# SonyCSLParis/audio-metrics

Hardware: AMD Instinct MI355X
Metric: evaluate() embeddings/sec (FAD+KD+PRDC), 2×100k CLAP-512 sets, 1/2/4/8 GPUs (higher is better)
Workload: dtype f32

## Files before the change

audio-metrics_amd/_lib.py:

```python
import ctypes
import os
from ctypes import c_char_p, c_double, c_int, c_int64, c_size_t, c_void_p

from ._build import DEV_LIB_PATH, LIB_PATH

_P = c_void_p

SIGNATURES = {
    "am_version": (c_char_p, []),
    "am_status_string": (c_char_p, [c_int]),
    "am_last_error": (c_char_p, []),
    "am_stats_workspace_bytes": (c_size_t, [c_int64, c_int]),
    "am_stats_f32": (c_int, [_P, c_int64, c_int, c_int64, _P, _P, _P, c_size_t, _P]),
    "am_colsum_f32": (c_int, [_P, c_int64, c_int, c_int64, _P, _P, c_size_t, _P]),
    "am_scatter_f32": (c_int, [_P, c_int64, c_int, c_int64, _P, _P, _P, c_size_t, _P]),
    "am_stats_f64_workspace_bytes": (c_size_t, [c_int64, c_int]),
    "am_stats_f64": (c_int, [_P, c_int64, c_int, c_int64, _P, _P, _P, c_size_t, _P]),
    "am_colsum_f64": (c_int, [_P, c_int64, c_int, c_int64, _P, _P, c_size_t, _P]),
    "am_scatter_f64": (c_int, [_P, c_int64, c_int, c_int64, _P, _P, _P, c_size_t, _P]),
    "am_stats_merge_f64": (c_int, [c_int64, _P, _P, c_int64, _P, _P, c_int, _P, _P, _P]),
    "am_stats_push_max_rows": (c_int, []),
    "am_stats_push_f32": (c_int, [_P, c_int64, c_int, c_int64, c_int64, _P, _P, _P, _P, c_int64, _P]),
    "am_frechet_workspace_bytes": (c_size_t, [c_int]),
    "am_frechet_f64": (c_int, [_P, _P, _P, _P, c_int, c_int, c_double, _P, _P, c_size_t, _P]),
    "am_frechet_first_block": (c_int, []),
    "am_frechet_enqueue_f64": (c_int, [_P, _P, _P, _P, c_int, c_int, c_int, c_int, c_double, _P, _P, c_size_t, _P]),
    "am_apa_f64": (c_double, [c_double, c_double, c_double]),
    "am_kd_workspace_bytes": (c_size_t, [c_int, c_int]),
    "am_kd_poly_workspace_bytes": (c_size_t, [c_int, c_int, c_int]),
    "am_kd_poly_f32": (c_int, [_P, c_int64, c_int64, _P, c_int64, c_int64, c_int, _P, _P, c_int, c_int,
                               c_double, c_double, c_int, _P, _P, c_size_t, _P]),
    "am_kd_draw_indices": (c_int, [ctypes.c_uint64, ctypes.c_uint64, ctypes.c_uint64, ctypes.c_uint64, c_int64, c_int64, c_int,
                                   c_int, _P, _P]),
    "am_kd_rbf_workspace_bytes": (c_size_t, [c_int, c_int]),
    "am_kd_rbf_f32": (c_int, [_P, c_int64, c_int64, _P, c_int64, c_int64, c_int, _P, _P, c_int, c_int, c_double, _P, _P,
                              c_size_t, _P]),
    "am_knn_workspace_bytes": (c_size_t, [c_int64, c_int64, c_int, c_int]),
    "am_knn_radii_f32": (c_int, [_P, c_int64, c_int64, _P, c_int64, c_int64, c_int, c_int, _P, _P, c_size_t, _P]),
    "am_knn_sym_eligible": (c_int, [c_int64, c_int, c_int]),
    "am_knn_list_width": (c_int, [c_int]),
    "am_knn_part_workspace_bytes": (c_size_t, [c_int64, c_int, c_int]),
    "am_knn_bounds_f32": (c_int, [_P, c_int64, c_int64, c_int, c_int, c_int64, c_int64, _P, _P, c_size_t, _P]),
    "am_knn_sym_part_f32": (c_int, [_P, c_int64, c_int64, c_int, c_int, c_int, c_int, _P, _P, _P, c_size_t, _P]),
    "am_knn_lists_finish_workspace_bytes": (c_size_t, [c_int64, c_int, c_int]),
    "am_knn_lists_finish_f32": (c_int, [_P, c_int, _P, c_int64, c_int64, c_int, c_int, _P, _P, c_size_t, _P]),
    "am_prdc_workspace_bytes": (c_size_t, [c_int64, c_int64, c_int]),
    "am_prdc_counts_f32": (c_int, [_P, c_int64, c_int64, _P, c_int64, c_int64, c_int, _P, _P, _P, _P, _P, _P,
                                   _P, c_size_t, _P]),
    "am_prdc_reduce": (c_int, [_P, c_int64, _P, _P, c_int64, _P, _P]),
    "am_prepared_half_ld": (c_int64, [c_int]),
    "am_prepare_set_f32": (c_int, [_P, c_int64, c_int64, c_int, _P, _P, _P, _P]),
    "am_knn_radii_prepared_f32": (c_int, [_P, c_int64, c_int64, c_int, _P, c_int, _P, _P, c_size_t, _P]),
    "am_knn_bounds_prepared_f32": (c_int, [_P, c_int64, c_int64, c_int, _P, c_int, c_int64, c_int64, _P, _P, c_size_t, _P]),
    "am_knn_sym_part_prepared_f32": (c_int, [_P, c_int64, c_int64, c_int, _P, c_int, c_int, c_int, _P, _P, _P, c_size_t, _P]),
    "am_prdc_counts_prepared_f32": (c_int, [_P, c_int64, c_int64, _P, _P, c_int64, c_int64, _P, c_int, _P, _P, _P, _P, _P, _P,
                                            _P, c_size_t, _P]),
    "am_knn_f64_workspace_bytes": (c_size_t, [c_int64, c_int64, c_int, c_int]),
    "am_knn_radii_f64": (c_int, [_P, c_int64, c_int64, _P, c_int64, c_int64, c_int, c_int, _P, _P, c_size_t, _P]),
    "am_prdc_f64_workspace_bytes": (c_size_t, [c_int64, c_int64, c_int]),
    "am_prdc_counts_f64": (c_int, [_P, c_int64, c_int64, _P, c_int64, c_int64, c_int, _P, _P, _P, _P, _P, _P,
                                   _P, c_size_t, _P]),
    "am_kd_f64_workspace_bytes": (c_size_t, [c_int, c_int]),
    "am_kd_poly_f64": (c_int, [_P, c_int64, c_int64, _P, c_int64, c_int64, c_int, _P, _P, c_int, c_int,
                               c_double, c_double, c_int, _P, _P, c_size_t, _P]),
    "am_kd_rbf_f64": (c_int, [_P, c_int64, c_int64, _P, c_int64, c_int64, c_int, _P, _P, c_int, c_int, c_double, _P, _P,
                              c_size_t, _P]),
    "am_eigh_workspace_bytes": (c_size_t, [c_int]),
    "am_eigh_sym_f64": (c_int, [_P, c_int, _P, _P, c_int, _P, c_size_t, _P]),
    "am_project_f64": (c_int, [_P, c_int64, c_int64, c_int, _P, _P, c_int, _P, _P]),
    "am_project_rows_f64": (c_int, [_P, c_int64, c_int64, c_int, _P, _P, c_int, _P, _P]),
    "am_evaluate_workspace_bytes": (c_size_t, [c_int64, c_int64, c_int, c_int, c_int, c_int, ctypes.c_uint]),
    "am_evaluate_f32": (c_int, [_P, c_int64, c_int64, _P, c_int64, c_int64, c_int, ctypes.c_uint, c_int, _P, _P, c_int, c_int,
                                c_double, c_double, c_int, _P, _P, _P, _P, c_size_t, _P, _P]),
    "am_evaluate_sharded_workspace_bytes": (c_size_t, [_P, _P, c_int, c_int, c_int, c_int, c_int, c_int, ctypes.c_uint]),
    "am_evaluate_sharded_f32": (c_int, [_P, c_int64, _P, c_int64, c_int, _P, _P, _P, ctypes.c_uint, c_int, _P, _P, c_int, c_int,
                                        c_double, c_double, c_int, _P, _P, c_size_t, _P, _P, _P]),
    "am_kernel_clock_enable": (c_int, [c_int]),
    "am_kernel_clock_read": (c_int, [c_int, _P, _P]),
    "am_knn_path": (c_int, [c_int64, c_int64, c_int, c_int, c_int]),
    "am_prdc_path": (c_int, [c_int64, c_int64, c_int]),
    "am_kd_path": (c_int, [c_int64, c_int64, c_int64, c_int64, c_int, c_int, c_int, c_int]),
    "am_filter_engine": (c_int, [c_int]),
    "am_filter_stats_enable": (c_int, [_P]),
}


class HipLibraryError(RuntimeError):
    pass


class PreparedSetStruct(ctypes.Structure):
    _fields_ = [("norms", c_void_p), ("stats", c_void_p), ("half", c_void_p)]


class EvaluateSideStruct(ctypes.Structure):
    _fields_ = [("mean", c_void_p), ("cov", c_void_p), ("radii", c_void_p),
                ("mean_out", c_void_p), ("cov_out", c_void_p), ("radii_out", c_void_p)]


ALL_REDUCE_SUM_FN = ctypes.CFUNCTYPE(c_int, c_void_p, c_void_p, c_int64, c_int, c_void_p)
ALL_GATHER_V_FN = ctypes.CFUNCTYPE(c_int, c_void_p, c_void_p, c_void_p, ctypes.POINTER(c_int64), c_void_p)


class CollectivesStruct(ctypes.Structure):
# ... 43 lines not shown
```

audio-metrics_amd/csrc/am_common.h:

```cpp
#pragma once
#include <hip/hip_runtime.h>
#include <stdint.h>
#include <stddef.h>
#include <stdio.h>
#include "../../include/audio_metrics_hip.h"

namespace am {

char* last_error_buf();
void set_error(const char* fmt, ...);

#define AM_HIP_TRY(expr)                                                             \
    do {                                                                             \
        hipError_t _e = (expr);                                                      \
        if (_e != hipSuccess) {                                                      \
            am::set_error("%s failed: %s (%s:%d)", #expr, hipGetErrorString(_e),     \
                          __FILE__, __LINE__);                                       \
            return AM_ERR_HIP;                                                       \
        }                                                                            \
    } while (0)

#define AM_LAUNCH_CHECK()                                                            \
    do {                                                                             \
        hipError_t _e = hipGetLastError();                                           \
        if (_e != hipSuccess) {                                                      \
            am::set_error("kernel launch failed: %s (%s:%d)", hipGetErrorString(_e), \
                          __FILE__, __LINE__);                                       \
            return AM_ERR_HIP;                                                       \
        }                                                                            \
    } while (0)

#define AM_REQUIRE(cond, status, ...)                                                \
    do {                                                                             \
        if (!(cond)) {                                                               \
            am::set_error(__VA_ARGS__);                                              \
            return (status);                                                         \
        }                                                                            \
    } while (0)

hipError_t ensure_dynamic_lds(const void* kernel, int bytes);

void clock_begin(int kernel, hipStream_t st);
void clock_end(int kernel, hipStream_t st);

__device__ __forceinline__ float clamp0(float v) { return v != v ? __builtin_inff() : fmaxf(v, 0.f); }

static inline bool aligned16(const void* p) { return (reinterpret_cast<uintptr_t>(p) & 15u) == 0; }
static inline size_t round_up(size_t x, size_t a) { return (x + a - 1) / a * a; }
static inline int64_t ceil_div(int64_t a, int64_t b) { return (a + b - 1) / b; }

struct Carver {
    char* base;
    size_t size;
    size_t off = 0;
    Carver(void* p, size_t n) : base(static_cast<char*>(p)), size(n) {}
    template <class T>
    T* take(size_t count) {
        size_t bytes = round_up(count * sizeof(T), 256);
        T* r = (base && off + bytes <= size) ? reinterpret_cast<T*>(base + off) : nullptr;
        off += bytes;
        return r;
    }
    bool ok() const { return base != nullptr && off <= size; }
};

bool knn64_filter_eligible(int64_t N, int D, int k);
size_t knn64_filter_workspace(int64_t N, int D, int k);
int knn64_filter(const double* X, int64_t N, int64_t ld, int D, int k, double* out_r, void* ws, size_t ws_bytes, hipStream_t st);
bool prdc64_filter_eligible(int64_t Nr, int64_t Nc, int D);
size_t prdc64_filter_workspace(int64_t Nr, int64_t Nc, int D);
int prdc64_filter(const double* R, int64_t Nr, int64_t ldr, const double* C, int64_t Nc, int64_t ldc, int D, const double* rt,
                  const double* ct, int32_t* col_count, unsigned* row_any, unsigned* row_cover, const int** fail_flag, void* ws,
                  size_t ws_bytes, hipStream_t st);
size_t knn64_self_workspace(int64_t N, int k);
int knn64_self_gated(const double* X, int64_t N, int64_t ld, int D, int k, double* out_r, void* ws, size_t ws_bytes, const int* run_flag,
                     hipStream_t st);


}
```

audio-metrics_amd/csrc/evaluate.hip:

```cpp
#include "am_common.h"
#include <algorithm>
#include <vector>

namespace am {

__global__ void eval_pack_kernel(const double* __restrict__ fad5, const long long* __restrict__ totals, double* __restrict__ out,
                                 unsigned what) {
    const int t = threadIdx.x;
    if (t < AM_EVAL_HEAD) {
        double v = 0.0;
        if (t < 5) v = (what & AM_EVAL_FAD) ? fad5[t] : (t == 4 ? -1.0 : 0.0);
        else if (t < 9) v = (what & AM_EVAL_PRDC) ? (double)totals[t - 5] : 0.0;
        out[t] = v;
    }
}

struct EvalLayout {
    size_t total = 0;
    size_t stats_ws = 0, knn_ws = 0, prdc_ws = 0, kd_ws = 0, fad_ws = 0;
    double *mean[2] = {nullptr, nullptr}, *cov[2] = {nullptr, nullptr};
    float *norms[2] = {nullptr, nullptr}, *radii[2] = {nullptr, nullptr};
    uint32_t* pstats[2] = {nullptr, nullptr};
    uint16_t* half[2] = {nullptr, nullptr};
    int32_t* col = nullptr;
// ... 32 lines not shown
        main_bytes = std::max({main_bytes, am_knn_workspace_bytes(n_ref, n_ref, D, k), am_knn_workspace_bytes(n_cand, n_cand, D, k),
                               am_prdc_workspace_bytes(n_ref, n_cand, D)});
    }
    if (what & AM_EVAL_KD) main_bytes = std::max(main_bytes, am_kd_poly_workspace_bytes(S, m, D));
    L.ws_main_bytes = round_up(std::max<size_t>(main_bytes, 256), 256);
    L.ws_main = c.take<char>(L.ws_main_bytes);
    L.total = c.off;
    return c.ok();
}

}

using namespace am;

extern "C" size_t am_evaluate_workspace_bytes(int64_t n_ref, int64_t n_cand, int D, int nearest_k, int kd_subsets, int kd_m,
                                              unsigned what) {
    if (n_ref < 1 || n_cand < 1 || D < 1) return 0;
    Carver c(nullptr, 0);
    EvalLayout L;
    eval_layout(c, n_ref, n_cand, D, nearest_k, kd_subsets, kd_m, what, L);
    return L.total;
}

extern "C" int am_evaluate_f32(const float* ref, int64_t n_ref, int64_t ld_ref, const float* cand, int64_t n_cand,
                               int64_t ld_cand, int D, unsigned what, int nearest_k, const int64_t* idx_cand,
                               const int64_t* idx_ref, int kd_subsets, int kd_m, double kd_gamma, double kd_coef0, int kd_degree,
                               const am_evaluate_side* given_ref, const am_evaluate_side* given_cand, double* out, void* ws,
                               size_t ws_bytes, am_stream_t stream, am_stream_t side_stream) {
    AM_REQUIRE(ref && cand && out, AM_ERR_BAD_ARG, "null pointer");
    AM_REQUIRE(n_ref >= 1 && n_cand >= 1 && D >= 1, AM_ERR_BAD_SHAPE, "sets of %lld and %lld rows x %d", (long long)n_ref,
               (long long)n_cand, D);
    AM_REQUIRE((what & ~(unsigned)(AM_EVAL_FAD | AM_EVAL_KD | AM_EVAL_PRDC)) == 0 && what != 0, AM_ERR_BAD_ARG, "what = %u", what);
    AM_REQUIRE(!(what & AM_EVAL_KD) || (idx_cand && idx_ref && kd_subsets >= 1 && kd_m >= 1), AM_ERR_BAD_ARG,
               "kernel distance needs the two index tables");
    AM_REQUIRE(!(what & AM_EVAL_FAD) || side_stream != stream, AM_ERR_BAD_ARG,
               "the Frechet solve runs on side_stream, which must differ from stream");
    hipStream_t st = static_cast<hipStream_t>(stream), side = static_cast<hipStream_t>(side_stream);
#ifdef AM_DEV_KNOBS
    static const int fad_place = getenv("AM_EVAL_FAD_PLACE") ? atoi(getenv("AM_EVAL_FAD_PLACE")) : 0;
#else
    constexpr int fad_place = 0;
#endif
    Carver c(ws, ws_bytes);
    EvalLayout L;
    AM_REQUIRE(eval_layout(c, n_ref, n_cand, D, nearest_k, kd_subsets, kd_m, what, L), AM_ERR_WORKSPACE,
               "workspace too small: need %zu bytes, have %zu", L.total, ws_bytes);
    const float* X[2] = {ref, cand};
    const int64_t n[2] = {n_ref, n_cand}, ld[2] = {ld_ref, ld_cand};
    const am_evaluate_side* given[2] = {given_ref, given_cand};
    int rc;

    const double* mean[2];
    const double* cov[2];
    if (what & AM_EVAL_FAD) {
        for (int s = 0; s < 2; ++s) {
            if (given[s] && given[s]->mean && given[s]->cov) {
                mean[s] = given[s]->mean;
                cov[s] = given[s]->cov;
                continue;
            }
            double* m_out = given[s] && given[s]->mean_out ? given[s]->mean_out : L.mean[s];
            double* c_out = given[s] && given[s]->cov_out ? given[s]->cov_out : L.cov[s];
            if ((rc = am_stats_f32(X[s], n[s], D, ld[s], m_out, c_out, L.ws_main, L.ws_main_bytes, stream)) != AM_OK) return rc;
            mean[s] = m_out;
            cov[s] = c_out;
        }
    }
    struct EventGuard {
        hipEvent_t e = nullptr;
        ~EventGuard() {
            if (e) (void)hipEventDestroy(e);
        }
    } ev_stats, ev_fad;
    if ((what & AM_EVAL_FAD) && fad_place != 2) {
        AM_HIP_TRY(hipEventCreateWithFlags(&ev_stats.e, hipEventDisableTiming));
        AM_HIP_TRY(hipEventRecord(ev_stats.e, st));
    }

    if (what & AM_EVAL_PRDC) {
        am_prepared_set prep[2];
        for (int s = 0; s < 2; ++s) {
            if ((rc = am_prepare_set_f32(X[s], n[s], ld[s], D, L.norms[s], L.pstats[s], L.half[s], stream)) != AM_OK) return rc;
            prep[s].norms = L.norms[s];
            prep[s].stats = L.pstats[s];
            prep[s].half = L.half[s];
        }
        const float* radii[2];
        for (int s = 0; s < 2; ++s) {
            if (given[s] && given[s]->radii) {
                radii[s] = given[s]->radii;
                continue;
            }
            float* r_out = given[s] && given[s]->radii_out ? given[s]->radii_out : L.radii[s];
            if ((rc = am_knn_radii_prepared_f32(X[s], n[s], ld[s], D, &prep[s], nearest_k, r_out, L.ws_main, L.ws_main_bytes,
                                                stream)) != AM_OK)
                return rc;
            radii[s] = r_out;
            if ((what & AM_EVAL_FAD) && fad_place == 2 && ev_stats.e == nullptr) {
                AM_HIP_TRY(hipEventCreateWithFlags(&ev_stats.e, hipEventDisableTiming));
                AM_HIP_TRY(hipEventRecord(ev_stats.e, st));
            }
        }
        if ((rc = am_prdc_counts_prepared_f32(ref, n_ref, ld_ref, &prep[0], cand, n_cand, ld_cand, &prep[1], D, radii[0], radii[1],
                                              L.col, L.rany, L.rcov, nullptr, L.ws_main, L.ws_main_bytes, stream)) != AM_OK)
            return rc;
        if ((rc = am_prdc_reduce(L.col, n_cand, L.rany, L.rcov, n_ref, reinterpret_cast<int64_t*>(L.totals), stream)) != AM_OK)
            return rc;
    }

    if (what & AM_EVAL_KD) {
        if ((rc = am_kd_poly_f32(cand, n_cand, ld_cand, ref, n_ref, ld_ref, D, idx_cand, idx_ref, kd_subsets, kd_m, kd_gamma,
                                 kd_coef0, kd_degree, out + AM_EVAL_HEAD, L.ws_main, L.ws_main_bytes, stream)) != AM_OK)
            return rc;
    }

    if (what & AM_EVAL_FAD) {
        const bool serial = fad_place == 1;
        if (!serial) {
            if (ev_stats.e == nullptr) {
                AM_HIP_TRY(hipEventCreateWithFlags(&ev_stats.e, hipEventDisableTiming));
                AM_HIP_TRY(hipEventRecord(ev_stats.e, st));
            }
            AM_HIP_TRY(hipStreamWaitEvent(side, ev_stats.e, 0));
        }
        const int block = am_frechet_first_block(), max_iter = 64;
        for (int first = 0; first < 2 * block; first += block)
            if ((rc = am_frechet_enqueue_f64(mean[1], cov[1], mean[0], cov[0], D, first, block, max_iter, 1e-13, L.fad_out,
                                             L.ws_fad, L.fad_ws, serial ? stream : side_stream)) != AM_OK)
                return rc;
        if (!serial) {
            AM_HIP_TRY(hipEventCreateWithFlags(&ev_fad.e, hipEventDisableTiming));
            AM_HIP_TRY(hipEventRecord(ev_fad.e, side));
            AM_HIP_TRY(hipStreamWaitEvent(st, ev_fad.e, 0));
        }
    }
// ... 358 lines not shown
```

audio-metrics_amd/csrc/pairwise.hip:

```cpp
#include "pairwise_common.h"
#include <algorithm>
#include <vector>
#include <cmath>
#include <type_traits>

namespace am {

__global__ void __launch_bounds__(256) row_sqnorm_kernel(const float* __restrict__ X, int64_t N, int64_t ld,
                                                         int D, float* __restrict__ out) {
    const int lane = threadIdx.x & 63;
    const int64_t row = (int64_t)blockIdx.x * 4 + (threadIdx.x >> 6);
    if (row >= N) return;
    const float* x = X + row * ld;
    float acc = 0.f;
    for (int k = lane * 4; k < D; k += 256) {
        const f32x4 v = load_k4(x, k, D);
        acc = fmaf(v.x, v.x, acc);
        acc = fmaf(v.y, v.y, acc);
        acc = fmaf(v.z, v.z, acc);
        acc = fmaf(v.w, v.w, acc);
    }
#pragma unroll
    for (int off = 32; off >= 1; off >>= 1) acc = acc + __shfl_xor(acc, off);
    if (lane == 0) out[row] = acc;
// ... 1261 lines not shown
    L.c32 = c.take<float>((size_t)Nc * L.ld32);
    L.rn = c.take<float>(Nr);
    L.rt = c.take<float>(Nr);
    L.cn = c.take<float>(Nc);
    L.ct = c.take<float>(Nc);
    L.rmin = c.take<unsigned>(Nr);
    L.plan = plan_cross_fast(Nr, Nc, D);
    L.buf = carve_cross_fast(c, Nr, Nc, D, L.plan);
    L.total = c.off;
    return c.ok();
}
size_t prdc64_filter_workspace(int64_t Nr, int64_t Nc, int D) {
    Carver c(nullptr, 0);
    Prdc64Layout L;
    prdc64_layout(c, Nr, Nc, D, L);
    return L.total;
}

int prdc64_filter(const double* R, int64_t Nr, int64_t ldr, const double* C, int64_t Nc, int64_t ldc, int D, const double* rt,
                  const double* ct, int32_t* col_count, unsigned* row_any, unsigned* row_cover, const int** fail_flag, void* ws,
                  size_t ws_bytes, hipStream_t st) {
    Carver c(ws, ws_bytes);
    Prdc64Layout L;
    AM_REQUIRE(prdc64_layout(c, Nr, Nc, D, L), AM_ERR_WORKSPACE, "workspace too small: need %zu bytes, have %zu", L.total, ws_bytes);
    hipLaunchKernelGGL(cast64_kernel, dim3((unsigned)ceil_div(Nr * L.ld32, 256)), dim3(256), 0, st, R, Nr, ldr, D, L.r32, L.ld32);
    hipLaunchKernelGGL(cast64_kernel, dim3((unsigned)ceil_div(Nc * L.ld32, 256)), dim3(256), 0, st, C, Nc, ldc, D, L.c32, L.ld32);
    hipLaunchKernelGGL(narrow64_kernel, dim3((unsigned)ceil_div(Nr, 256)), dim3(256), 0, st, rt, Nr, L.rt);
    hipLaunchKernelGGL(narrow64_kernel, dim3((unsigned)ceil_div(Nc, 256)), dim3(256), 0, st, ct, Nc, L.ct);
    hipLaunchKernelGGL(fill_u32_kernel, dim3((unsigned)ceil_div(Nr, 256)), dim3(256), 0, st, L.rmin, Nr, 0x7f800000u);
    AM_LAUNCH_CHECK();
    int rc;
    if ((rc = norms_of(nullptr, L.r32, Nr, L.ld32, D, L.rn, st)) != AM_OK) return rc;
    if ((rc = norms_of(nullptr, L.c32, Nc, L.ld32, D, L.cn, st)) != AM_OK) return rc;
    const Prdc64Hook h{R, C, ldr, ldc, rt, ct};
    if ((rc = run_cross_fast(L.r32, Nr, L.ld32, L.rn, L.rt, L.c32, Nc, L.ld32, L.cn, L.ct, D, L.plan, L.buf, col_count, L.rmin, row_any,
                             row_cover, false, st, nullptr, nullptr, &h)) != AM_OK)
        return rc;
    *fail_flag = L.buf.ov_count + 1;
    return AM_OK;
}

}

extern "C" int am_knn_radii_f32(const float* X, int64_t N, int64_t ldx, const float* Y, int64_t M, int64_t ldy,
                                int D, int k, float* out_r, void* ws, size_t ws_bytes, am_stream_t stream) {
    return knn_radii_impl(X, N, ldx, Y, M, ldy, D, k, out_r, ws, ws_bytes, stream, nullptr);
}

static bool prepared_ok(const am_prepared_set* p) { return p != nullptr && p->norms != nullptr && p->stats != nullptr && p->half != nullptr; }
static PreparedSet prepared_of(const am_prepared_set* p) { return PreparedSet{p->norms, p->stats, p->half}; }

extern "C" int64_t am_prepared_half_ld(int D) { return D < 1 ? 0 : half_ld(D); }

extern "C" int am_prepare_set_f32(const float* X, int64_t N, int64_t ld, int D, float* norms, uint32_t* stats4, uint16_t* half,
                                  am_stream_t stream) {
    int rc;
    if ((rc = check_matrix(X, N, ld, D, "X")) != AM_OK) return rc;
    AM_REQUIRE(norms && stats4 && half, AM_ERR_BAD_ARG, "null output pointer");
    hipStream_t st = static_cast<hipStream_t>(stream);
    if ((rc = launch_norms(X, N, ld, D, norms, st)) != AM_OK) return rc;
    AM_HIP_TRY(hipMemsetAsync(stats4, 0, 4 * sizeof(unsigned), st));
    return launch_to_half(X, N, ld, D, norms, stats4, 0, half, st);
}

extern "C" int am_knn_radii_prepared_f32(const float* X, int64_t N, int64_t ldx, int D, const am_prepared_set* prepared, int k,
                                         float* out_r, void* ws, size_t ws_bytes, am_stream_t stream) {
    AM_REQUIRE(prepared_ok(prepared), AM_ERR_BAD_ARG, "prepared set has a null member");
    const PreparedSet ps = prepared_of(prepared);
    return knn_radii_impl(X, N, ldx, X, N, ldx, D, k, out_r, ws, ws_bytes, stream, &ps);
}

extern "C" int am_filter_stats_enable(int64_t* device_slots) {
    if (device_slots == nullptr) {
        g_filter_stats = nullptr;
        g_filter_stats_device = -1;
        return AM_OK;
    }
    int dev = -1;
    AM_HIP_TRY(hipGetDevice(&dev));
    g_filter_stats = reinterpret_cast<long long*>(device_slots);
    g_filter_stats_device = dev;
    return AM_OK;
}

extern "C" int am_knn_path(int64_t N, int64_t M, int D, int k, int self) {
    if (N < 1 || M < 1 || D < 1 || k < 1) return -1;
    if (k > AM_MAX_K) return 4;
    const KnnPlan p = plan_knn(N, M, D, k, self != 0 && N == M);
    return !p.sym ? 0 : (knn_fast_enabled(N, D) ? (p.tile_rows == 256 ? 3 : 2) : 1);
}
extern "C" int am_prdc_path(int64_t Nr, int64_t Nc, int D) {
    if (Nr < 1 || Nc < 1 || D < 1) return -1;
    if (!cross_fast_enabled(Nr, Nc, D)) return 0;
    return plan_cross_fast(Nr, Nc, D).wide ? 3 : 2;
}

extern "C" int am_filter_engine(int D) {
    if (D < 1) return 0;
    const int Dh = (int)(half_ld(D) / 2);
    return wide_stationary(Dh) ? (pstat64_supported(Dh) ? 2 : 1) : 0;
}

extern "C" int am_knn_sym_eligible(int64_t N, int D, int k) {
    if (N < 1 || D < 1 || k < 1 || k > AM_MAX_K) return 0;
    return plan_knn(N, N, D, k, true).sym ? 1 : 0;
}

extern "C" int am_knn_list_width(int k) { return (k < 1 || k > AM_MAX_K) ? 0 : kcap_for(k + 1); }

extern "C" size_t am_knn_part_workspace_bytes(int64_t N, int D, int k) {
    if (N < 1 || D < 1 || k < 1 || k > AM_MAX_K) return 0;
    const KnnPlan p = plan_knn(N, N, D, k, true, true);
    Carver c(nullptr, 0);
    KnnBuffers b;
    carve_knn(c, N, N, p, b);
// ... 313 lines not shown
```

audio-metrics_amd/csrc/stats.hip:

```cpp
#include "am_common.h"
#include "tile_engine.h"
#include <algorithm>

namespace am {

constexpr int SC_ROWS = 32;
constexpr int SC_LD = 128;
constexpr int SC_SLAB = SC_ROWS * SC_LD;
constexpr int SC_FLUSH = 8;

__global__ void __launch_bounds__(256) colsum_partial_kernel(const float* __restrict__ X, int64_t N, int64_t ld,
                                                             int D, int64_t rows_per_block,
                                                             double* __restrict__ partial) {
    __shared__ double red[256 * 4];
    const int tid = threadIdx.x;
    const int cgs = (D + 3) / 4;
    const int cpp = cgs < 256 ? cgs : 256;
    const int rpar = 256 / cpp;
    const int my_cg = tid % cpp, my_r = tid / cpp;
    const int64_t r0 = (int64_t)blockIdx.x * rows_per_block;
    const int64_t r1 = (r0 + rows_per_block < N) ? r0 + rows_per_block : N;
    for (int cg0 = 0; cg0 < cgs; cg0 += cpp) {
        const int cg = cg0 + my_cg;
        double s0 = 0, s1 = 0, s2 = 0, s3 = 0;
// ... 260 lines not shown
        mu[which][c] = s / (double)b;
    }
    __syncthreads();
    for (int e = tid; e < b * PUSH_TILE; e += 256) {
        const int r = e / PUSH_TILE, c = e % PUSH_TILE;
        ea[r][c] -= (float)mu[0][c];
        eb[r][c] -= (float)mu[1][c];
    }
    __syncthreads();
    const double n1 = (double)n_old, n2 = (double)b, n = n1 + n2;
    const int c = tid % PUSH_TILE;
#pragma unroll
    for (int q = 0; q < PUSH_TILE / 8; ++q) {
        const int r = tid / PUSH_TILE + 8 * q;
        const int gi = i0 + r, gj = j0 + c;
        if (gi >= D || gj >= D) continue;
        double sum = 0;
        for (int k = 0; k < b; ++k) sum = fma((double)ea[k][r], (double)eb[k][c], sum);
        const double cov2 = b > 1 ? sum / (double)(b - 1) : 0.0;
        const int64_t o = (int64_t)gi * D + gj;
        if (n_old == 0) {
            cov[o] = cov2;
        } else {
            const double w1 = (n1 - 1) / (n - 1), w2 = (n2 - 1) / (n - 1), wd = (n1 * n2 / n) / (n - 1);
            const double di = mean_in[gi] - mu[0][r], dj = mean_in[gj] - mu[1][c];
            cov[o] = (w1 * cov[o] + w2 * cov2) + wd * (di * dj);
        }
    }
    if (ti == tj && tid < PUSH_TILE && i0 + tid < D) {
        const int g = i0 + tid;
        mean_out[g] = n_old == 0 ? mu[0][tid] : (n1 * mean_in[g] + n2 * mu[0][tid]) / n;
    }
    if (rows_out != nullptr) {
        const int64_t total = (int64_t)b * D;
        const int64_t nwg = (int64_t)gridDim.x * gridDim.y, wg = (int64_t)ti * gridDim.x + tj;
        const int64_t per = (total + nwg - 1) / nwg;
        const int64_t lo = wg * per, hi = lo + per < total ? lo + per : total;
        for (int64_t e = lo + tid; e < hi; e += 256) {
            const int64_t r = e / D, col = e % D;
            rows_out[r * ld_out + col] = E[r * ld + col];
        }
    }
}

struct StatsPlan {
    int cs_blocks;
    int64_t cs_rows;
    int ntri, nslabs;
    int64_t slab_rows;
};

static StatsPlan plan_stats(int64_t N, int D) {
    StatsPlan p;
    int64_t b = ceil_div(N, 64);
    if (b > 512) b = 512;
    if (b < 1) b = 1;
    p.cs_rows = ceil_div(N, b);
    p.cs_blocks = (int)ceil_div(N, p.cs_rows);
    const int T = (int)ceil_div(D, TB);
    p.ntri = T * (T + 1) / 2;
    int64_t s = std::max<int64_t>(512 / p.ntri, 1);
    const int64_t max_s = ceil_div(N, SC_ROWS * SC_FLUSH);
    if (s > max_s) s = max_s;
    if (s < 1) s = 1;
    p.slab_rows = ceil_div(ceil_div(N, s), SC_ROWS) * SC_ROWS;
    p.nslabs = (int)ceil_div(N, p.slab_rows);
    return p;
}

static size_t stats_ws(int64_t N, int D, const StatsPlan& p) {
    Carver c(nullptr, 0);
    c.take<double>((size_t)p.cs_blocks * D);
    c.take<double>((size_t)p.nslabs * p.ntri * TB * TB);
    c.take<double>(D);
    return c.off;
}

static int check_x(const float* X, int64_t N, int D, int64_t ld) {
    AM_REQUIRE(X != nullptr, AM_ERR_BAD_ARG, "X is null");
    AM_REQUIRE(N >= 1 && D >= 1, AM_ERR_BAD_SHAPE, "X has shape %lld x %d", (long long)N, D);
    AM_REQUIRE(aligned16(X) && ld % 4 == 0 && ld >= D, AM_ERR_BAD_ARG,
               "X must be 16-byte aligned with ld %% 4 == 0 and ld >= D (ld=%lld, D=%d)", (long long)ld, D);
    return AM_OK;
}

constexpr int S64_TILE = 32;
__global__ void __launch_bounds__(256) colsum64_partial_kernel(const double* __restrict__ X, int64_t N, int64_t ld, int D,
                                                               int64_t rows_per_block, double* __restrict__ partial) {
    const int64_t r0 = (int64_t)blockIdx.x * rows_per_block;
    const int64_t r1 = (r0 + rows_per_block < N) ? r0 + rows_per_block : N;
    for (int d = threadIdx.x; d < D; d += 256) {
        double s = 0.0;
        for (int64_t row = r0; row < r1; ++row) s += X[row * ld + d];
        partial[(int64_t)blockIdx.x * D + d] = s;
    }
}

__global__ void __launch_bounds__(256) scatter64_partial_kernel(const double* __restrict__ X, int64_t N, int64_t ld, int D,
                                                                const double* __restrict__ mean, int64_t slab_rows, int ntri,
                                                                double* __restrict__ partial) {
    const int T = (D + S64_TILE - 1) / S64_TILE;
    int tp, tq;
    tri_decode((int)(blockIdx.x % ntri), T, tp, tq);
    const int64_t slab = blockIdx.x / ntri;
    const int lane = threadIdx.x & 63, wave = threadIdx.x >> 6;
    const int l15 = lane & 15, l4 = lane >> 4;
    const int ca = tp * S64_TILE + (wave >> 1) * 16 + l15, cb = tq * S64_TILE + (wave & 1) * 16 + l15;
    const double ma = ca < D ? mean[ca] : 0.0, mb = cb < D ? mean[cb] : 0.0;
    const int64_t r0 = slab * slab_rows;
    const int64_t r1 = (r0 + slab_rows < N) ? r0 + slab_rows : N;
    typedef double f64x4s __attribute__((ext_vector_type(4)));
// ... 64 lines not shown
    AM_LAUNCH_CHECK();
    return AM_OK;
}

static int run_scatter(const float* X, int64_t N, int D, int64_t ld, const double* mean, double scale, double* out,
                       double* partial, const StatsPlan& p, hipStream_t st) {
    if (D % TB == 0)
        hipLaunchKernelGGL(scatter_partial_kernel<true>, dim3((unsigned)(p.ntri * p.nslabs)), dim3(ENGINE_THREADS), 0, st, X, N, ld,
                           D, mean, p.slab_rows, p.ntri, partial);
    else
        hipLaunchKernelGGL(scatter_partial_kernel<false>, dim3((unsigned)(p.ntri * p.nslabs)), dim3(ENGINE_THREADS), 0, st, X, N, ld,
                           D, mean, p.slab_rows, p.ntri, partial);
    AM_LAUNCH_CHECK();
    hipLaunchKernelGGL(scatter_reduce_kernel, dim3((unsigned)(TB * TB / 256), (unsigned)p.ntri), dim3(256), 0, st, partial,
                       p.nslabs, p.ntri, D, scale, out);
    AM_LAUNCH_CHECK();
    return AM_OK;
}

}

using namespace am;

extern "C" size_t am_stats_workspace_bytes(int64_t N, int D) {
    if (N < 1 || D < 1) return 0;
    return stats_ws(N, D, plan_stats(N, D));
}

extern "C" int am_colsum_f32(const float* X, int64_t N, int D, int64_t ld, double* colsum, void* ws, size_t ws_bytes,
                             am_stream_t stream) {
    int rc;
    if ((rc = check_x(X, N, D, ld)) != AM_OK) return rc;
    AM_REQUIRE(colsum != nullptr, AM_ERR_BAD_ARG, "colsum is null");
    const StatsPlan p = plan_stats(N, D);
    Carver c(ws, ws_bytes);
    double* cs_part = c.take<double>((size_t)p.cs_blocks * D);
    AM_REQUIRE(c.ok(), AM_ERR_WORKSPACE, "workspace too small: need %zu bytes, have %zu", c.off, ws_bytes);
    return run_colsum(X, N, D, ld, 1.0, colsum, cs_part, p, static_cast<hipStream_t>(stream));
}

extern "C" int am_scatter_f32(const float* X, int64_t N, int D, int64_t ld, const double* mean, double* scatter,
                              void* ws, size_t ws_bytes, am_stream_t stream) {
    int rc;
    if ((rc = check_x(X, N, D, ld)) != AM_OK) return rc;
    AM_REQUIRE(mean && scatter, AM_ERR_BAD_ARG, "mean/scatter is null");
    const StatsPlan p = plan_stats(N, D);
    Carver c(ws, ws_bytes);
    c.take<double>((size_t)p.cs_blocks * D);
    double* sc_part = c.take<double>((size_t)p.nslabs * p.ntri * TB * TB);
    AM_REQUIRE(c.ok(), AM_ERR_WORKSPACE, "workspace too small: need %zu bytes, have %zu", c.off, ws_bytes);
    return run_scatter(X, N, D, ld, mean, 1.0, scatter, sc_part, p, static_cast<hipStream_t>(stream));
}

extern "C" int am_stats_f32(const float* X, int64_t N, int D, int64_t ld, double* mean, double* cov, void* ws,
                            size_t ws_bytes, am_stream_t stream) {
    int rc;
    if ((rc = check_x(X, N, D, ld)) != AM_OK) return rc;
    AM_REQUIRE(mean && cov, AM_ERR_BAD_ARG, "mean/cov is null");
    hipStream_t st = static_cast<hipStream_t>(stream);
    const StatsPlan p = plan_stats(N, D);
    Carver c(ws, ws_bytes);
    double* cs_part = c.take<double>((size_t)p.cs_blocks * D);
    double* sc_part = c.take<double>((size_t)p.nslabs * p.ntri * TB * TB);
    AM_REQUIRE(c.ok(), AM_ERR_WORKSPACE, "workspace too small: need %zu bytes, have %zu", c.off, ws_bytes);
    if ((rc = run_colsum(X, N, D, ld, 1.0 / (double)N, mean, cs_part, p, st)) != AM_OK) return rc;
    if (N == 1) {
        hipLaunchKernelGGL(zero_f64_kernel, dim3((unsigned)ceil_div((int64_t)D * D, 256)), dim3(256), 0, st, cov,
                           (int64_t)D * D);
        AM_LAUNCH_CHECK();
        return AM_OK;
    }
    return run_scatter(X, N, D, ld, mean, 1.0 / (double)(N - 1), cov, sc_part, p, st);
}

extern "C" size_t am_stats_f64_workspace_bytes(int64_t N, int D) {
    if (N < 1 || D < 1) return 0;
    return stats64_ws(D, plan_stats64(N, D));
}

static int check_x64(const double* X, int64_t N, int D, int64_t ld) {
    AM_REQUIRE(X != nullptr, AM_ERR_BAD_ARG, "X is null");
    AM_REQUIRE(N >= 1 && D >= 1, AM_ERR_BAD_SHAPE, "X has shape %lld x %d", (long long)N, D);
    AM_REQUIRE(D <= 8192, AM_ERR_BAD_SHAPE, "float64 statistics take rows of up to 8192 elements (D=%d)", D);
    AM_REQUIRE(ld >= D, AM_ERR_BAD_ARG, "ld=%lld < D=%d", (long long)ld, D);
    return AM_OK;
}

static int run_colsum64(const double* X, int64_t N, int D, int64_t ld, double scale, double* out, double* cs_part, const Stats64Plan& p,
                        hipStream_t st) {
    hipLaunchKernelGGL(colsum64_partial_kernel, dim3(p.cs_blocks), dim3(256), 0, st, X, N, ld, D, p.cs_rows, cs_part);
    AM_LAUNCH_CHECK();
    hipLaunchKernelGGL(colsum_reduce_kernel, dim3((unsigned)ceil_div(D, CSR_COLS)), dim3(256), 0, st, cs_part, p.cs_blocks, D, scale, out);
    AM_LAUNCH_CHECK();
    return AM_OK;
}

static int run_scatter64(const double* X, int64_t N, int D, int64_t ld, const double* mean, double scale, double* out, double* sc_part,
                         const Stats64Plan& p, hipStream_t st) {
    hipLaunchKernelGGL(scatter64_partial_kernel, dim3((unsigned)(p.ntri * p.nslabs)), dim3(256), 0, st, X, N, ld, D, mean, p.slab_rows,
                       p.ntri, sc_part);
    AM_LAUNCH_CHECK();
    hipLaunchKernelGGL(scatter64_reduce_kernel, dim3(S64_TILE * S64_TILE / 256, (unsigned)p.ntri), dim3(256), 0, st, sc_part,
                       p.nslabs, p.ntri, D, scale, out);
    AM_LAUNCH_CHECK();
    return AM_OK;
}

extern "C" int am_colsum_f64(const double* X, int64_t N, int D, int64_t ld, double* colsum, void* ws, size_t ws_bytes, am_stream_t stream) {
    int rc;
    if ((rc = check_x64(X, N, D, ld)) != AM_OK) return rc;
    AM_REQUIRE(colsum != nullptr, AM_ERR_BAD_ARG, "colsum is null");
    const Stats64Plan p = plan_stats64(N, D);
    Carver c(ws, ws_bytes);
    double* cs_part = c.take<double>((size_t)p.cs_blocks * D);
    AM_REQUIRE(c.ok(), AM_ERR_WORKSPACE, "workspace too small: need %zu bytes, have %zu", c.off, ws_bytes);
    return run_colsum64(X, N, D, ld, 1.0, colsum, cs_part, p, static_cast<hipStream_t>(stream));
}

extern "C" int am_scatter_f64(const double* X, int64_t N, int D, int64_t ld, const double* mean, double* scatter, void* ws, size_t ws_bytes,
                              am_stream_t stream) {
    int rc;
    if ((rc = check_x64(X, N, D, ld)) != AM_OK) return rc;
    AM_REQUIRE(mean && scatter, AM_ERR_BAD_ARG, "mean/scatter is null");
    const Stats64Plan p = plan_stats64(N, D);
    Carver c(ws, ws_bytes);
// ... 58 lines not shown
```

include/audio_metrics_hip.h:

```cpp
#ifndef AUDIO_METRICS_HIP_H
#define AUDIO_METRICS_HIP_H

#include <stddef.h>
#include <stdint.h>

#ifdef __cplusplus
extern "C" {
#endif

typedef void* am_stream_t;

typedef enum am_status {
    AM_OK = 0,
    AM_ERR_BAD_ARG = -1,
    AM_ERR_BAD_SHAPE = -2,
    AM_ERR_UNSUPPORTED_K = -3,
    AM_ERR_WORKSPACE = -4,
    AM_ERR_NO_CONVERGENCE = -5,
    AM_ERR_HIP = -6
} am_status;

#define AM_MAX_K 31

const char* am_version(void);
// ... 30 lines not shown
int am_frechet_f64(const double* mu_x, const double* cov_x,
                   const double* mu_y, const double* cov_y, int D,
                   int max_iter, double tol, double* out_host,
                   void* ws, size_t ws_bytes, am_stream_t stream);
int am_frechet_first_block(void);
int am_frechet_enqueue_f64(const double* mu_x, const double* cov_x,
                           const double* mu_y, const double* cov_y, int D,
                           int first_iter, int n_iter, int max_iter, double tol, double* out_dev,
                           void* ws, size_t ws_bytes, am_stream_t stream);

double am_apa_f64(double d_y_x, double d_y_xp, double d_x_xp);

size_t am_kd_workspace_bytes(int S, int m);
size_t am_kd_poly_workspace_bytes(int S, int m, int D);
int am_kd_poly_f32(const float* X, int64_t N1, int64_t ldx,
                   const float* Y, int64_t N2, int64_t ldy, int D,
                   const int64_t* idx1, const int64_t* idx2, int S, int m,
                   double gamma, double coef0, int degree,
                   double* out_mmd, void* ws, size_t ws_bytes, am_stream_t stream);

int am_kd_draw_indices(uint64_t state_hi, uint64_t state_lo, uint64_t inc_hi, uint64_t inc_lo,
                       int64_t n1, int64_t n2, int S, int m, int64_t* idx1, int64_t* idx2);

size_t am_kd_rbf_workspace_bytes(int S, int m);
int am_kd_rbf_f32(const float* X, int64_t N1, int64_t ldx,
                  const float* Y, int64_t N2, int64_t ldy, int D,
                  const int64_t* idx1, const int64_t* idx2, int S, int m, double sigma,
                  double* out_mmd, void* ws, size_t ws_bytes, am_stream_t stream);

size_t am_knn_workspace_bytes(int64_t N, int64_t M, int D, int k);
int am_knn_radii_f32(const float* X, int64_t N, int64_t ldx,
                     const float* Y, int64_t M, int64_t ldy, int D, int k,
                     float* out_r, void* ws, size_t ws_bytes, am_stream_t stream);

int am_knn_sym_eligible(int64_t N, int D, int k);
int am_knn_list_width(int k);
size_t am_knn_part_workspace_bytes(int64_t N, int D, int k);
int am_knn_bounds_f32(const float* X, int64_t N, int64_t ld, int D, int k, int64_t row0, int64_t nrows,
                      float* out_bound_sq, void* ws, size_t ws_bytes, am_stream_t stream);
int am_knn_sym_part_f32(const float* X, int64_t N, int64_t ld, int D, int k, int part, int nparts,
                        float* bounds_sq, float* out_lists, void* ws, size_t ws_bytes, am_stream_t stream);
size_t am_knn_lists_finish_workspace_bytes(int64_t N, int D, int k);
int am_knn_lists_finish_f32(const float* lists, int nparts, const float* X, int64_t N, int64_t ld, int D, int k,
                            float* out_r, void* ws, size_t ws_bytes, am_stream_t stream);

typedef struct am_prepared_set {
    const float* norms;
    const uint32_t* stats;
    const uint16_t* half;
} am_prepared_set;
int64_t am_prepared_half_ld(int D);
int am_prepare_set_f32(const float* X, int64_t N, int64_t ld, int D, float* norms, uint32_t* stats4, uint16_t* half,
                       am_stream_t stream);
int am_knn_radii_prepared_f32(const float* X, int64_t N, int64_t ldx, int D, const am_prepared_set* prepared, int k,
                              float* out_r, void* ws, size_t ws_bytes, am_stream_t stream);
int am_knn_bounds_prepared_f32(const float* X, int64_t N, int64_t ld, int D, const am_prepared_set* prepared, int k,
                               int64_t row0, int64_t nrows, float* out_bound_sq, void* ws, size_t ws_bytes, am_stream_t stream);
int am_knn_sym_part_prepared_f32(const float* X, int64_t N, int64_t ld, int D, const am_prepared_set* prepared, int k,
                                 int part, int nparts, float* bounds_sq, float* out_lists, void* ws, size_t ws_bytes,
                                 am_stream_t stream);
int am_prdc_counts_prepared_f32(const float* R, int64_t Nr, int64_t ldr, const am_prepared_set* prepared_r,
                                const float* C, int64_t Nc, int64_t ldc, const am_prepared_set* prepared_c, int D,
                                const float* r_ref, const float* r_cand,
                                int32_t* out_col_count, uint8_t* out_row_any, uint8_t* out_row_cover, float* out_row_min,
                                void* ws, size_t ws_bytes, am_stream_t stream);

size_t am_prdc_workspace_bytes(int64_t Nr, int64_t Nc, int D);
int am_prdc_counts_f32(const float* R, int64_t Nr, int64_t ldr,
                       const float* C, int64_t Nc, int64_t ldc, int D,
                       const float* r_ref, const float* r_cand,
                       int32_t* out_col_count, uint8_t* out_row_any, uint8_t* out_row_cover, float* out_row_min,
                       void* ws, size_t ws_bytes, am_stream_t stream);
int am_prdc_reduce(const int32_t* col_count, int64_t Nc,
                   const uint8_t* row_any, const uint8_t* row_cover, int64_t Nr,
                   int64_t* out4, am_stream_t stream);

size_t am_knn_f64_workspace_bytes(int64_t N, int64_t M, int D, int k);
int am_knn_radii_f64(const double* X, int64_t N, int64_t ldx,
                     const double* Y, int64_t M, int64_t ldy, int D, int k,
                     double* out_r, void* ws, size_t ws_bytes, am_stream_t stream);
size_t am_prdc_f64_workspace_bytes(int64_t Nr, int64_t Nc, int D);
int am_prdc_counts_f64(const double* R, int64_t Nr, int64_t ldr,
                       const double* C, int64_t Nc, int64_t ldc, int D,
                       const double* r_ref, const double* r_cand,
                       int32_t* out_col_count, uint8_t* out_row_any, uint8_t* out_row_cover, double* out_row_min,
                       void* ws, size_t ws_bytes, am_stream_t stream);
size_t am_kd_f64_workspace_bytes(int S, int m);
int am_kd_poly_f64(const double* X, int64_t N1, int64_t ldx,
                   const double* Y, int64_t N2, int64_t ldy, int D,
                   const int64_t* idx1, const int64_t* idx2, int S, int m,
                   double gamma, double coef0, int degree,
                   double* out_mmd, void* ws, size_t ws_bytes, am_stream_t stream);
int am_kd_rbf_f64(const double* X, int64_t N1, int64_t ldx,
                  const double* Y, int64_t N2, int64_t ldy, int D,
                  const int64_t* idx1, const int64_t* idx2, int S, int m, double sigma,
                  double* out_mmd, void* ws, size_t ws_bytes, am_stream_t stream);

size_t am_eigh_workspace_bytes(int D);
int am_eigh_sym_f64(const double* A, int D, double* evals, double* evecs, int max_sweeps,
                    void* ws, size_t ws_bytes, am_stream_t stream);
int am_project_f64(const float* X, int64_t N, int64_t ld, int D, const double* mean, const double* components, int p,
                   double* out, am_stream_t stream);
int am_project_rows_f64(const double* X, int64_t N, int64_t ld, int D, const double* mean, const double* components, int p,
                        double* out, am_stream_t stream);

#define AM_EVAL_FAD 1u
// ... 50 lines not shown
```

Baseline: 8.758 million.

## Fuse row norms, abs-max stats and column sums into one prepare pass

Adds a fused kernel that, in one read of X, computes row norms, max-norm and max-abs statistics, and per-block column sums. evaluate() now produces the FAD mean and the PRDC preparation data from this single pass, and the standalone prepare path also uses it. This is meant to remove redundant full passes over the 100k×512 embedding matrices (separate colsum, norms and stats scans). The trade-offs are extra code paths, plus double-precision accumulation and LDS reduction work inside the fused kernel.

```diff
diff --git a/audio-metrics_amd/_lib.py b/audio-metrics_amd/_lib.py
--- a/audio-metrics_amd/_lib.py
+++ b/audio-metrics_amd/_lib.py
@@ -50,6 +50,8 @@
     "am_prdc_reduce": (c_int, [_P, c_int64, _P, _P, c_int64, _P, _P]),
     "am_prepared_half_ld": (c_int64, [c_int]),
     "am_prepare_set_f32": (c_int, [_P, c_int64, c_int64, c_int, _P, _P, _P, _P]),
+    "am_prepare_set_separate_f32": (c_int, [_P, c_int64, c_int64, c_int, _P, _P, _P, _P]),
+    "am_prepare_stats_f32": (c_int, [_P, c_int64, c_int64, c_int, _P, _P, _P, _P, c_size_t, _P]),
     "am_knn_radii_prepared_f32": (c_int, [_P, c_int64, c_int64, c_int, _P, c_int, _P, _P, c_size_t, _P]),
     "am_knn_bounds_prepared_f32": (c_int, [_P, c_int64, c_int64, c_int, _P, c_int, c_int64, c_int64, _P, _P, c_size_t, _P]),
     "am_knn_sym_part_prepared_f32": (c_int, [_P, c_int64, c_int64, c_int, _P, c_int, c_int, c_int, _P, _P, _P, c_size_t, _P]),
diff --git a/audio-metrics_amd/csrc/am_common.h b/audio-metrics_amd/csrc/am_common.h
--- a/audio-metrics_amd/csrc/am_common.h
+++ b/audio-metrics_amd/csrc/am_common.h
@@ -64,6 +64,13 @@
     bool ok() const { return base != nullptr && off <= size; }
 };
 
+void colsum_plan(int64_t N, int64_t* rows_per_block, int* blocks);
+bool prepare_fused_applies(int D);
+int launch_prepare_fused(const float* X, int64_t N, int64_t ld, int D, float* norms, unsigned* stats, double* partial, hipStream_t st);
+int stats_prepare_f32(const float* X, int64_t N, int D, int64_t ld, double* mean, double* cov, float* norms, unsigned* stats4, void* ws,
+                      size_t ws_bytes, hipStream_t st);
+int prepare_half(const float* X, int64_t N, int64_t ld, int D, const unsigned* stats4, uint16_t* half, hipStream_t st);
+
 bool knn64_filter_eligible(int64_t N, int D, int k);
 size_t knn64_filter_workspace(int64_t N, int D, int k);
 int knn64_filter(const double* X, int64_t N, int64_t ld, int D, int k, double* out_r, void* ws, size_t ws_bytes, hipStream_t st);
diff --git a/audio-metrics_amd/csrc/evaluate.hip b/audio-metrics_amd/csrc/evaluate.hip
--- a/audio-metrics_amd/csrc/evaluate.hip
+++ b/audio-metrics_amd/csrc/evaluate.hip
@@ -108,6 +108,7 @@
 
     const double* mean[2];
     const double* cov[2];
+    bool prepared_early[2] = {false, false};
     if (what & AM_EVAL_FAD) {
         for (int s = 0; s < 2; ++s) {
             if (given[s] && given[s]->mean && given[s]->cov) {
@@ -117,7 +118,14 @@
             }
             double* m_out = given[s] && given[s]->mean_out ? given[s]->mean_out : L.mean[s];
             double* c_out = given[s] && given[s]->cov_out ? given[s]->cov_out : L.cov[s];
-            if ((rc = am_stats_f32(X[s], n[s], D, ld[s], m_out, c_out, L.ws_main, L.ws_main_bytes, stream)) != AM_OK) return rc;
+            if ((what & AM_EVAL_PRDC) && prepare_fused_applies(D)) {
+                if ((rc = stats_prepare_f32(X[s], n[s], D, ld[s], m_out, c_out, L.norms[s], L.pstats[s], L.ws_main, L.ws_main_bytes,
+                                            st)) != AM_OK)
+                    return rc;
+                prepared_early[s] = true;
+            } else if ((rc = am_stats_f32(X[s], n[s], D, ld[s], m_out, c_out, L.ws_main, L.ws_main_bytes, stream)) != AM_OK) {
+                return rc;
+            }
             mean[s] = m_out;
             cov[s] = c_out;
         }
@@ -136,7 +144,9 @@
     if (what & AM_EVAL_PRDC) {
         am_prepared_set prep[2];
         for (int s = 0; s < 2; ++s) {
-            if ((rc = am_prepare_set_f32(X[s], n[s], ld[s], D, L.norms[s], L.pstats[s], L.half[s], stream)) != AM_OK) return rc;
+            rc = prepared_early[s] ? prepare_half(X[s], n[s], ld[s], D, L.pstats[s], L.half[s], st)
+                                   : am_prepare_set_f32(X[s], n[s], ld[s], D, L.norms[s], L.pstats[s], L.half[s], stream);
+            if (rc != AM_OK) return rc;
             prep[s].norms = L.norms[s];
             prep[s].stats = L.pstats[s];
             prep[s].half = L.half[s];
diff --git a/audio-metrics_amd/csrc/pairwise.hip b/audio-metrics_amd/csrc/pairwise.hip
--- a/audio-metrics_amd/csrc/pairwise.hip
+++ b/audio-metrics_amd/csrc/pairwise.hip
@@ -1337,15 +1337,40 @@
 
 extern "C" int64_t am_prepared_half_ld(int D) { return D < 1 ? 0 : half_ld(D); }
 
+static int prepare_set_separate(const float* X, int64_t N, int64_t ld, int D, float* norms, uint32_t* stats4, uint16_t* half,
+                                hipStream_t st) {
+    int rc;
+    if ((rc = launch_norms(X, N, ld, D, norms, st)) != AM_OK) return rc;
+    AM_HIP_TRY(hipMemsetAsync(stats4, 0, 4 * sizeof(unsigned), st));
+    return launch_to_half(X, N, ld, D, norms, stats4, 0, half, st);
+}
+
+int am::prepare_half(const float* X, int64_t N, int64_t ld, int D, const unsigned* stats4, uint16_t* half, hipStream_t st) {
+    const int64_t ldh = half_ld(D);
+    hipLaunchKernelGGL(to_half_kernel, dim3((unsigned)ceil_div(N * (ldh / 8), 256)), dim3(256), 0, st, X, N, ld, D, ldh, stats4 + 2,
+                       half, half_drop_bits());
+    AM_LAUNCH_CHECK();
+    return AM_OK;
+}
+
 extern "C" int am_prepare_set_f32(const float* X, int64_t N, int64_t ld, int D, float* norms, uint32_t* stats4, uint16_t* half,
                                   am_stream_t stream) {
     int rc;
     if ((rc = check_matrix(X, N, ld, D, "X")) != AM_OK) return rc;
     AM_REQUIRE(norms && stats4 && half, AM_ERR_BAD_ARG, "null output pointer");
     hipStream_t st = static_cast<hipStream_t>(stream);
-    if ((rc = launch_norms(X, N, ld, D, norms, st)) != AM_OK) return rc;
+    if (!prepare_fused_applies(D)) return prepare_set_separate(X, N, ld, D, norms, stats4, half, st);
     AM_HIP_TRY(hipMemsetAsync(stats4, 0, 4 * sizeof(unsigned), st));
-    return launch_to_half(X, N, ld, D, norms, stats4, 0, half, st);
+    if ((rc = launch_prepare_fused(X, N, ld, D, norms, stats4, nullptr, st)) != AM_OK) return rc;
+    return prepare_half(X, N, ld, D, stats4, half, st);
+}
+
+extern "C" int am_prepare_set_separate_f32(const float* X, int64_t N, int64_t ld, int D, float* norms, uint32_t* stats4,
+                                           uint16_t* half, am_stream_t stream) {
+    int rc;
+    if ((rc = check_matrix(X, N, ld, D, "X")) != AM_OK) return rc;
+    AM_REQUIRE(norms && stats4 && half, AM_ERR_BAD_ARG, "null output pointer");
+    return prepare_set_separate(X, N, ld, D, norms, stats4, half, static_cast<hipStream_t>(stream));
 }
 
 extern "C" int am_knn_radii_prepared_f32(const float* X, int64_t N, int64_t ldx, int D, const am_prepared_set* prepared, int k,
diff --git a/audio-metrics_amd/csrc/prepare_fused.hip b/audio-metrics_amd/csrc/prepare_fused.hip
--- /dev/null
+++ b/audio-metrics_amd/csrc/prepare_fused.hip
@@ -0,0 +1,146 @@
+#include "am_common.h"
+#include "tile_engine.h"
+#include <algorithm>
+
+namespace am {
+
+void colsum_plan(int64_t N, int64_t* rows_per_block, int* blocks) {
+    int64_t b = ceil_div(N, 64);
+    if (b > 512) b = 512;
+    if (b < 1) b = 1;
+    *rows_per_block = ceil_div(N, b);
+    *blocks = (int)ceil_div(N, *rows_per_block);
+}
+
+constexpr int PF_MAX_DIM = 4096;
+constexpr int PF_LDS_DOUBLES = 1024;
+
+template <int NT, int U>
+__global__ void __launch_bounds__(256) prepare_fused_kernel(const float* __restrict__ X, int64_t N, int64_t ld, int D,
+                                                            int64_t rows_per_block, int rpar, float* __restrict__ norms,
+                                                            unsigned* __restrict__ stats, double* __restrict__ partial) {
+    __shared__ double red[PF_LDS_DOUBLES];
+    __shared__ unsigned wave_max[2][4];
+    const int lane = threadIdx.x & 63, wave = threadIdx.x >> 6, nwaves = blockDim.x >> 6;
+    const int64_t r0 = (int64_t)blockIdx.x * rows_per_block;
+    const int64_t r1 = (r0 + rows_per_block < N) ? r0 + rows_per_block : N;
+    const bool sums = partial != nullptr;
+    unsigned m_abs = 0u, m_norm = 0u;
+
+    auto row_norm = [&](const f32x4 (&v)[NT]) {
+        float acc = 0.f;
+#pragma unroll
+        for (int t = 0; t < NT; ++t) {
+            acc = fmaf(v[t].x, v[t].x, acc);
+            acc = fmaf(v[t].y, v[t].y, acc);
+            acc = fmaf(v[t].z, v[t].z, acc);
+            acc = fmaf(v[t].w, v[t].w, acc);
+            m_abs = max(max(m_abs, __float_as_uint(v[t].x) & 0x7fffffffu), __float_as_uint(v[t].y) & 0x7fffffffu);
+            m_abs = max(max(m_abs, __float_as_uint(v[t].z) & 0x7fffffffu), __float_as_uint(v[t].w) & 0x7fffffffu);
+        }
+#pragma unroll
+        for (int off = 32; off >= 1; off >>= 1) acc = acc + __shfl_xor(acc, off);
+        return acc;
+    };
+
+    for (int rr = wave; rr < rpar; rr += nwaves) {
+        double s[NT][4];
+#pragma unroll
+        for (int t = 0; t < NT; ++t)
+#pragma unroll
+            for (int e = 0; e < 4; ++e) s[t][e] = 0.0;
+        int64_t row = r0 + rr;
+        for (; row + (int64_t)(U - 1) * rpar < r1; row += (int64_t)U * rpar) {
+            f32x4 v[U][NT];
+#pragma unroll
+            for (int u = 0; u < U; ++u)
+#pragma unroll
+                for (int t = 0; t < NT; ++t) v[u][t] = load_k4(X + (row + (int64_t)u * rpar) * ld, (lane + 64 * t) * 4, D);
+#pragma unroll
+            for (int u = 0; u < U; ++u) {
+                const float nrm = row_norm(v[u]);
+                m_norm = max(m_norm, __float_as_uint(nrm));
+                if (lane == 0) norms[row + (int64_t)u * rpar] = nrm;
+#pragma unroll
+                for (int t = 0; t < NT; ++t)
+#pragma unroll
+                    for (int e = 0; e < 4; ++e) s[t][e] += (double)v[u][t][e];
+            }
+        }
+        for (; row < r1; row += rpar) {
+            f32x4 v[NT];
+#pragma unroll
+            for (int t = 0; t < NT; ++t) v[t] = load_k4(X + row * ld, (lane + 64 * t) * 4, D);
+            const float nrm = row_norm(v);
+            m_norm = max(m_norm, __float_as_uint(nrm));
+            if (lane == 0) norms[row] = nrm;
+#pragma unroll
+            for (int t = 0; t < NT; ++t)
+#pragma unroll
+                for (int e = 0; e < 4; ++e) s[t][e] += (double)v[t][e];
+        }
+        if (sums) {
+            double* dst = rpar == 1 ? partial + (int64_t)blockIdx.x * D : red + (int64_t)rr * (((D + 3) / 4) * 4);
+#pragma unroll
+            for (int t = 0; t < NT; ++t)
+#pragma unroll
+                for (int e = 0; e < 4; ++e) {
+                    const int c = (lane + 64 * t) * 4 + e;
+                    if (c < D) dst[c] = s[t][e];
+                }
+        }
+    }
+#pragma unroll
+    for (int off = 32; off >= 1; off >>= 1) m_abs = max(m_abs, (unsigned)__shfl_xor((int)m_abs, off));
+    if (lane == 0) {
+        wave_max[0][wave] = m_norm;
+        wave_max[1][wave] = m_abs;
+    }
+    __syncthreads();
+    if (sums && rpar > 1) {
+        const int dp = ((D + 3) / 4) * 4;
+        for (int c = threadIdx.x; c < D; c += blockDim.x) {
+            double t = red[c];
+            for (int rr = 1; rr < rpar; ++rr) t += red[rr * dp + c];
+            partial[(int64_t)blockIdx.x * D + c] = t;
+        }
+    }
+    if (threadIdx.x == 0) {
+        unsigned a = 0u, b = 0u;
+        for (int w = 0; w < nwaves; ++w) {
+            a = max(a, wave_max[0][w]);
+            b = max(b, wave_max[1][w]);
+        }
+        if (a != 0u) atomicMax(stats + 0, a);
+        if (b != 0u) atomicMax(stats + 2, b);
+    }
+}
+
+bool prepare_fused_applies(int D) { return D >= 1 && D <= PF_MAX_DIM; }
+
+int launch_prepare_fused(const float* X, int64_t N, int64_t ld, int D, float* norms, unsigned* stats, double* partial,
+                         hipStream_t st) {
+    AM_REQUIRE(prepare_fused_applies(D), AM_ERR_BAD_SHAPE, "the fused preparation pass takes rows of up to %d elements (D=%d)",
+               PF_MAX_DIM, D);
+    int64_t rows;
+    int blocks;
+    colsum_plan(N, &rows, &blocks);
+    const int cgs = (D + 3) / 4;
+    const int cpp = cgs < 256 ? cgs : 256;
+    const int rpar = 256 / cpp;
+    const dim3 grid((unsigned)blocks), block(64u * (unsigned)std::min(rpar, 4));
+#define AM_PF_LAUNCH(NT, U)                                                                                                   \
+    hipLaunchKernelGGL((prepare_fused_kernel<NT, U>), grid, block, 0, st, X, N, ld, D, rows, rpar, norms, stats, partial)
+    const int nt = (int)ceil_div(cgs, 64);
+    if (nt <= 1) AM_PF_LAUNCH(1, 8);
+    else if (nt <= 2) AM_PF_LAUNCH(2, 8);
+    else if (nt <= 3) AM_PF_LAUNCH(3, 4);
+    else if (nt <= 4) AM_PF_LAUNCH(4, 4);
+    else if (nt <= 8) AM_PF_LAUNCH(8, 2);
+    else AM_PF_LAUNCH(16, 1);
+#undef AM_PF_LAUNCH
+    AM_LAUNCH_CHECK();
+    return AM_OK;
+}
+
+}
diff --git a/audio-metrics_amd/csrc/stats.hip b/audio-metrics_amd/csrc/stats.hip
--- a/audio-metrics_amd/csrc/stats.hip
+++ b/audio-metrics_amd/csrc/stats.hip
@@ -336,11 +336,7 @@
 
 static StatsPlan plan_stats(int64_t N, int D) {
     StatsPlan p;
-    int64_t b = ceil_div(N, 64);
-    if (b > 512) b = 512;
-    if (b < 1) b = 1;
-    p.cs_rows = ceil_div(N, b);
-    p.cs_blocks = (int)ceil_div(N, p.cs_rows);
+    colsum_plan(N, &p.cs_rows, &p.cs_blocks);
     const int T = (int)ceil_div(D, TB);
     p.ntri = T * (T + 1) / 2;
     int64_t s = std::max<int64_t>(512 / p.ntri, 1);
@@ -511,18 +507,25 @@
     return run_scatter(X, N, D, ld, mean, 1.0, scatter, sc_part, p, static_cast<hipStream_t>(stream));
 }
 
-extern "C" int am_stats_f32(const float* X, int64_t N, int D, int64_t ld, double* mean, double* cov, void* ws,
-                            size_t ws_bytes, am_stream_t stream) {
+static int stats_impl(const float* X, int64_t N, int D, int64_t ld, double* mean, double* cov, float* norms, unsigned* stats4,
+                      void* ws, size_t ws_bytes, hipStream_t st) {
     int rc;
     if ((rc = check_x(X, N, D, ld)) != AM_OK) return rc;
     AM_REQUIRE(mean && cov, AM_ERR_BAD_ARG, "mean/cov is null");
-    hipStream_t st = static_cast<hipStream_t>(stream);
     const StatsPlan p = plan_stats(N, D);
     Carver c(ws, ws_bytes);
     double* cs_part = c.take<double>((size_t)p.cs_blocks * D);
     double* sc_part = c.take<double>((size_t)p.nslabs * p.ntri * TB * TB);
     AM_REQUIRE(c.ok(), AM_ERR_WORKSPACE, "workspace too small: need %zu bytes, have %zu", c.off, ws_bytes);
-    if ((rc = run_colsum(X, N, D, ld, 1.0 / (double)N, mean, cs_part, p, st)) != AM_OK) return rc;
+    if (norms != nullptr) {
+        AM_HIP_TRY(hipMemsetAsync(stats4, 0, 4 * sizeof(unsigned), st));
+        if ((rc = launch_prepare_fused(X, N, ld, D, norms, stats4, cs_part, st)) != AM_OK) return rc;
+        hipLaunchKernelGGL(colsum_reduce_kernel, dim3((unsigned)ceil_div(D, CSR_COLS)), dim3(256), 0, st, cs_part, p.cs_blocks, D,
+                           1.0 / (double)N, mean);
+        AM_LAUNCH_CHECK();
+    } else if ((rc = run_colsum(X, N, D, ld, 1.0 / (double)N, mean, cs_part, p, st)) != AM_OK) {
+        return rc;
+    }
     if (N == 1) {
         hipLaunchKernelGGL(zero_f64_kernel, dim3((unsigned)ceil_div((int64_t)D * D, 256)), dim3(256), 0, st, cov,
                            (int64_t)D * D);
@@ -530,6 +533,40 @@
         return AM_OK;
     }
     return run_scatter(X, N, D, ld, mean, 1.0 / (double)(N - 1), cov, sc_part, p, st);
+}
+
+int am::stats_prepare_f32(const float* X, int64_t N, int D, int64_t ld, double* mean, double* cov, float* norms, unsigned* stats4,
+                          void* ws, size_t ws_bytes, hipStream_t st) {
+    AM_REQUIRE(norms && stats4, AM_ERR_BAD_ARG, "null output pointer");
+    return stats_impl(X, N, D, ld, mean, cov, norms, stats4, ws, ws_bytes, st);
+}
+
+extern "C" int am_stats_f32(const float* X, int64_t N, int D, int64_t ld, double* mean, double* cov, void* ws,
+                            size_t ws_bytes, am_stream_t stream) {
+    return stats_impl(X, N, D, ld, mean, cov, nullptr, nullptr, ws, ws_bytes, static_cast<hipStream_t>(stream));
+}
+
+extern "C" int am_prepare_stats_f32(const float* X, int64_t N, int64_t ld, int D, float* norms, uint32_t* stats4, double* colsum,
+                                    void* ws, size_t ws_bytes, am_stream_t stream) {
+    int rc;
+    if ((rc = check_x(X, N, D, ld)) != AM_OK) return rc;
+    AM_REQUIRE(norms && stats4, AM_ERR_BAD_ARG, "null output pointer");
+    hipStream_t st = static_cast<hipStream_t>(stream);
+    const StatsPlan p = plan_stats(N, D);
+    double* cs_part = nullptr;
+    if (colsum != nullptr) {
+        Carver c(ws, ws_bytes);
+        cs_part = c.take<double>((size_t)p.cs_blocks * D);
+        AM_REQUIRE(c.ok(), AM_ERR_WORKSPACE, "workspace too small: need %zu bytes, have %zu", c.off, ws_bytes);
+    }
+    AM_HIP_TRY(hipMemsetAsync(stats4, 0, 4 * sizeof(unsigned), st));
+    if ((rc = launch_prepare_fused(X, N, ld, D, norms, stats4, cs_part, st)) != AM_OK) return rc;
+    if (colsum != nullptr) {
+        hipLaunchKernelGGL(colsum_reduce_kernel, dim3((unsigned)ceil_div(D, CSR_COLS)), dim3(256), 0, st, cs_part, p.cs_blocks, D, 1.0,
+                           colsum);
+        AM_LAUNCH_CHECK();
+    }
+    return AM_OK;
 }
 
 extern "C" size_t am_stats_f64_workspace_bytes(int64_t N, int D) {
diff --git a/include/audio_metrics_hip.h b/include/audio_metrics_hip.h
--- a/include/audio_metrics_hip.h
+++ b/include/audio_metrics_hip.h
@@ -106,6 +106,10 @@
 int64_t am_prepared_half_ld(int D);
 int am_prepare_set_f32(const float* X, int64_t N, int64_t ld, int D, float* norms, uint32_t* stats4, uint16_t* half,
                        am_stream_t stream);
+int am_prepare_set_separate_f32(const float* X, int64_t N, int64_t ld, int D, float* norms, uint32_t* stats4, uint16_t* half,
+                                am_stream_t stream);
+int am_prepare_stats_f32(const float* X, int64_t N, int64_t ld, int D, float* norms, uint32_t* stats4, double* colsum,
+                         void* ws, size_t ws_bytes, am_stream_t stream);
 int am_knn_radii_prepared_f32(const float* X, int64_t N, int64_t ldx, int D, const am_prepared_set* prepared, int k,
                               float* out_r, void* ws, size_t ws_bytes, am_stream_t stream);
 int am_knn_bounds_prepared_f32(const float* X, int64_t N, int64_t ld, int D, const am_prepared_set* prepared, int k,
```

Result: no change. 8.824 million (median of 6 runs) (+0.8%).
